# tjhladish/PLS

Hardware: AMD Instinct MI355X
Metric: NIPALS components/sec (higher is better)
Workload: dtype f64; 1 GPU; C3: synthetic tall n=1048576 x p=512, m=1, A=20, f64, resident in HBM; algo=nipals, fuse=1, deflation_written_back_every=1, rows_per_gpu=1048576, parallelism=single GPU

## Files before the change

pls_amd/csrc/ctx.hpp:

```cpp
#pragma once

namespace {

struct DevBuf {
    void *p = nullptr;
    size_t bytes = 0;
};

struct Launch {
    int fam;
    i64 bytes;
    hipEvent_t e0, e1;
};

}

struct pls_hip_context {
    int device = 0;
    hipStream_t stream = nullptr;
    pls_hip_allreduce_fn reducer = nullptr;
    void *reducer_user = nullptr;
    int rank = 0, nranks = 1;
    double *user_red = nullptr;
    i64 user_red_count = 0;
// ... 17 lines not shown
    i64 opt_val_lds_rows = -1;
    i64 val_lds_rows_dev = -1;
    std::string err;
    std::vector<hipEvent_t> ev_pool;
    size_t ev_used = 0;
    std::vector<Launch> launches;
    std::vector<Launch> fits;
    Launch cur_fit{};
    bool fit_timed = false;
    int num_cu = 256;
    plsh::Stager stager;
    int copy_threads = 0;
    hipStream_t copy_stream = nullptr;
    const double *pre_xx = nullptr, *pre_xy = nullptr;
    bool defer_free = false;
    std::vector<void *> graveyard;
    struct XchgIpc *xchg = nullptr;
    struct XchgEndpoint {
        bool on = false;
        int n = 0, rank = 0;
        double *const *inbox = nullptr;
        unsigned long long *const *flags = nullptr;
        unsigned long long *seq = nullptr;
        int *status = nullptr, *host_status = nullptr;
        const long long *limit = nullptr;
    } xep;
    DevBuf tailcnt;
    DevBuf resident;
    DevBuf rgflags;
    unsigned rg_epoch = 0;
    unsigned long long resident_launches = 0;
    struct Env {
        bool turnaround = true;
        i64 turn_edge_bytes = plsk::TURN_EDGE_BYTES;
        bool batch_refit = false;
        i64 batch_round = 0;
        i64 dualcv_round = 0;
        i64 dualbatch_round = 0;
        i64 resample_round = 0;
        bool resample_refit = false;
        bool dualbatch_sweeps = false;
        bool cvbatch_refit = false;
        i64 dualcvb_round = 0;
        i64 misscv_round = 0;
        bool tiny = true, cv_refit = false, tail = true, replica_guard = true, resident = true;
        int tail_update = 1;
        int xb4 = 1;
        int resident_gram = 1;
    };
    static void read_env(Env &env) {
        auto off = [](const char *name) { const char *e = getenv(name); return e && atoi(e) == 0; };
        auto on = [](const char *name) { const char *e = getenv(name); return e && atoi(e) != 0; };
        auto num = [](const char *name, i64 &v) { if (const char *e = getenv(name)) v = atoll(e); };
        env.tiny = !off("PLS_HIP_TINY");
        env.cv_refit = on("PLS_HIP_CV_REFIT");
        env.batch_refit = on("PLS_HIP_BATCH_REFIT");
        num("PLS_HIP_BATCH_ROUND", env.batch_round);
        num("PLS_HIP_DUALCV_ROUND", env.dualcv_round);
        num("PLS_HIP_DUALBATCH_ROUND", env.dualbatch_round);
        num("PLS_HIP_RESAMPLE_ROUND", env.resample_round);
        env.resample_refit = on("PLS_HIP_RESAMPLE_REFIT");
        env.dualbatch_sweeps = on("PLS_HIP_DUALBATCH_SWEEPS");
        env.cvbatch_refit = on("PLS_HIP_CVBATCH_REFIT");
        num("PLS_HIP_DUALCVB_ROUND", env.dualcvb_round);
        num("PLS_HIP_MISSCV_ROUND", env.misscv_round);
        env.tail = !off("PLS_HIP_TAIL");
        const char *tail = getenv("PLS_HIP_TAIL");
        env.tail_update = tail ? (atoi(tail) >= 2 ? 2 : 0) : 1;
        env.replica_guard = !off("PLS_HIP_REPLICA_GUARD");
        env.resident = !off("PLS_HIP_RESIDENT");
        env.turnaround = !off("PLS_HIP_TURNAROUND");
#ifdef PLS_HIP_TESTING
        num("PLS_HIP_TEST_TURN_EDGE_BYTES", env.turn_edge_bytes);
#endif
        if (const char *e = getenv("PLS_HIP_XB4")) env.xb4 = atoi(e);
        if (const char *e = getenv("PLS_HIP_RESIDENT_GRAM")) env.resident_gram = atoi(e);
    }
    Env env;
    int *diverged = nullptr, *diverged_dev = nullptr;
    DevBuf guard;
#ifdef PLS_HIP_TESTING
    int poison_new = -1;
#endif
};

#define PLS_HIP_WORKSPACES(SCRATCH, STATEFUL)                                                                                        \
    STATEFUL(zeros, WS_ALL, "256 zero bytes, cleared once when first used and only read afterwards: the source of out-of-range rows of the LDS-DMA panels") \
    STATEFUL(resident, 256, "two arrival counters of the resident fits, used in alternating parity (resident_launches): each launch zeroes the counter of the next; the payload behind the 256 bytes is scratch") \
    STATEFUL(rgflags, WS_ALL, "one arrival word per workgroup of resident_gram_fit_kernel: values only grow, a launch waits for words beyond rg_epoch, which the host advances by 4 per launch") \
    STATEFUL(gxx, c->pre_xx ? WS_ALL : 0, "X^T X accumulated during an upload, only while pre_xx points into it: from upload_accumulate to the end of the same host-memory fit") \
    STATEFUL(gxy, c->pre_xy ? WS_ALL : 0, "X^T Y accumulated during an upload, only while pre_xy points into it: from upload_accumulate to the end of the same host-memory fit") \
    SCRATCH(tailcnt) SCRATCH(part) SCRATCH(sspart) SCRATCH(xbpart) SCRATCH(wide1) SCRATCH(red) SCRATCH(red2) SCRATCH(xx) SCRATCH(xyp)  \
    SCRATCH(praw) SCRATCH(xy) SCRATCH(v) SCRATCH(cs) SCRATCH(coop) SCRATCH(lm) SCRATCH(tab) SCRATCH(work)                              \
    SCRATCH(cvidx) SCRATCH(cvx) SCRATCH(cvy) SCRATCH(cvws) SCRATCH(cve) SCRATCH(cvtx) SCRATCH(cvty) SCRATCH(cvtt) SCRATCH(cvm)         \
    SCRATCH(cvkeep) SCRATCH(cvred)                                                                                                     \
    SCRATCH(hX) SCRATCH(hY) SCRATCH(hT) SCRATCH(hW) SCRATCH(hP) SCRATCH(hQ) SCRATCH(hR) SCRATCH(hB) SCRATCH(hIn) SCRATCH(hOut)         \
    SCRATCH(valout) SCRATCH(valpart) SCRATCH(vale) SCRATCH(valacc) SCRATCH(valkeys) SCRATCH(valhist)                                   \
    SCRATCH(xdS) SCRATCH(xdQ) SCRATCH(xdPT) SCRATCH(xdred) SCRATCH(xdtv) SCRATCH(xdoQ) SCRATCH(xdoT) SCRATCH(xdoS) SCRATCH(xdsmall)    \
    SCRATCH(bws) SCRATCH(bv) SCRATCH(bred) SCRATCH(bmsg) SCRATCH(bssy) SCRATCH(bY) SCRATCH(boR) SCRATCH(boQ) SCRATCH(bott)             \
    SCRATCH(boB) SCRATCH(bossy)                                                                                                        \
    SCRATCH(dG) SCRATCH(dpart) SCRATCH(dV) SCRATCH(dT) SCRATCH(dY) SCRATCH(dZ) SCRATCH(dC) SCRATCH(dscr) SCRATCH(dcv) SCRATCH(dbat)    \
    SCRATCH(dcvb) SCRATCH(cvbpos) SCRATCH(cvbidx) SCRATCH(cvbo) SCRATCH(cvboE)                                                         \
    SCRATCH(rsw) SCRATCH(rsB) SCRATCH(rsacc) SCRATCH(rsX) SCRATCH(rsY) SCRATCH(rsW) SCRATCH(rsoS)                                      \
    SCRATCH(mX) SCRATCH(mws) SCRATCH(mit) SCRATCH(mzo) SCRATCH(mcv) SCRATCH(mcvidx)                                                    \
    SCRATCH(guard)

namespace {

constexpr size_t WS_ALL = ~(size_t)0;

template <typename F>
void for_each_workspace(pls_hip_context *c, F &&f) {
#define PLS_HIP_WS_SCRATCH(name) f(c->name, (size_t)0);
#define PLS_HIP_WS_STATEFUL(name, keep, reason) f(c->name, (size_t)(keep));
    PLS_HIP_WORKSPACES(PLS_HIP_WS_SCRATCH, PLS_HIP_WS_STATEFUL)
// ... 129 lines not shown
```

pls_amd/csrc/fused_kernels.hpp:

```cpp
#pragma once
#include <type_traits>

#include "common.hpp"
#include "exchange_kernels.hpp"
#include "update_m1.hpp"

namespace plsk {

#ifdef PLS_HIP_TESTING
__device__ unsigned long long *g_pass_stamps = nullptr;
#define PLS_STAMP(slot)                                                                                 \
    do {                                                                                                \
        if (g_pass_stamps && threadIdx.x == 0) {                                                        \
            g_pass_stamps[(size_t)blockIdx.x * 8 + (slot)] = wall_clock64();                            \
            if ((slot) == 0) {         \
                g_pass_stamps[(size_t)blockIdx.x * 8 + 4] = __builtin_amdgcn_s_getreg((31 << 11) | 20);  \
                g_pass_stamps[(size_t)blockIdx.x * 8 + 5] = __builtin_amdgcn_s_getreg((31 << 11) | 4);   \
            }                                                                                           \
        }                                                                                               \
    } while (0)
#else
#define PLS_STAMP(slot) do { } while (0)
#endif

// ... 34 lines not shown
template <typename T, int V>
__device__ __forceinline__ Pack<T, V> ld_pack_u(const T *p) {
    Pack<T, V> o;
    __builtin_memcpy(&o, p, sizeof(o));
    return o;
}
template <typename T, int V>
__device__ __forceinline__ void st_pack_u(T *p, const Pack<T, V> &x) {
    __builtin_memcpy(p, &x, sizeof(x));
}

template <typename T>
__device__ __forceinline__ __amdgpu_buffer_rsrc_t score_rsrc(const T *col, i64 nvalid) {
    return __builtin_amdgcn_make_buffer_rsrc(const_cast<T *>(col), (short)0, (int)(nvalid * (i64)sizeof(T)), BUF_WORD3);
}

struct TailUpdate {
    double *XY = nullptr;
    double *W = nullptr, *P = nullptr, *Q = nullptr, *R = nullptr, *vnext = nullptr;
    int A = 0, a = 0, nipals = 0;
};

struct WalkWeights {
    int nfull = -1;
    unsigned mask = 0;
    int rev = 0;
    int edge = 0;
};

struct Turn {
    bool on = false;
    bool rev = false;
    i64 edge_bytes = 0;
};

#ifdef PLS_HIP_TESTING
struct TurnRecord {
    int rev = 0, edge = 0, ntiles = 0, grid = 0;
};
inline TurnRecord g_test_turn;
#endif

struct SliceTail {
    unsigned *cnt = nullptr;
    double *red = nullptr;
    int nrows = 0;
    int npush = 0;
    unsigned long long seq = 0;
    XchgPeers peers;
    TailUpdate upd;
    XchgGather gx;
};

constexpr int TAIL_MIN_WG = 32;
constexpr int TAIL_AUX_SYS = 17;

__device__ __noinline__ void tail_update_m1(const double *src, i64 stride, int n, int sys, int ok, double *XY, double *W, double *P,
                                            double *Q, double *R, double *vnext, int K, int A, int a, int nipals, double *scratch,
                                            double *wl) {
    typedef unsigned int u32x2 __attribute__((ext_vector_type(2)));
    static_assert(XCHG_MAX == 2 * RED_SLICES, "two batches of RED_SLICES loads");
    const int L = K + 1;
    update_m1<512, 1>(
        [&](int j) -> double {
            double sum = 0.0;
#pragma unroll
// ... 129 lines not shown
    }
    if (!st.upd.XY) return;
    const TailUpdate &u = st.upd;
    if (st.gx.n > 0) {
        const XchgGather &gx = st.gx;
        if (tid == 0) *role = (*gx.status == 0);
        __syncthreads();
        if (tid < gx.n && *role) {
            const long long t0 = wall_clock64();
            while (__hip_atomic_load(gx.flags + tid, __ATOMIC_RELAXED, __HIP_MEMORY_SCOPE_SYSTEM) < gx.seq) {
                if (wall_clock64() - t0 > gx.limit) {
                    *role = 0;
                    break;
                }
                __builtin_amdgcn_s_sleep(4);
            }
            __builtin_amdgcn_fence(__ATOMIC_ACQUIRE, "");
            asm volatile("s_waitcnt vmcnt(0)" ::: "memory");
        }
        __syncthreads();
        const int ok = *role;
        if (!ok && tid == 0) {
            *gx.status = 1;
            __hip_atomic_store(gx.host_status, 1, __ATOMIC_RELAXED, __HIP_MEMORY_SCOPE_SYSTEM);
        }
        tail_update_m1(gx.inbox, gx.cap, gx.n, 1, ok, u.XY, u.W, u.P, u.Q, u.R, u.vnext, K, u.A, u.a, u.nipals, scratch, wl);
        return;
    }
    tail_update_m1(st.red, LP, RED_SLICES, 0, 1, u.XY, u.W, u.P, u.Q, u.R, u.vnext, K, u.A, u.a, u.nipals, scratch, wl);
}

constexpr int AUX_NT = 2;
constexpr i64 TURN_EDGE_BYTES = 192ll << 20;
constexpr bool TURN_LEAD_ST_DEFAULT = true;

template <bool XCD, int R>
struct TileWalk {
    __device__ __forceinline__ explicit TileWalk(i64) {}
    __device__ __forceinline__ unsigned first() const { return blockIdx.x; }
    __device__ __forceinline__ unsigned step() const { return gridDim.x; }
    __device__ __forceinline__ i64 nlim(i64 N) const { return N; }
};
template <int R>
struct TileWalk<true, R> {
    i64 first_, step_, nlim_;
    __device__ __forceinline__ explicit TileWalk(i64 N) : first_(blockIdx.x), step_(gridDim.x), nlim_(N) {
        if ((gridDim.x & 7) == 0) {
            const i64 per = ((N + R - 1) / R + 7) / 8;
            first_ = (i64)(blockIdx.x & 7) * per + (blockIdx.x >> 3);
            step_ = gridDim.x >> 3;
            nlim_ = min(N, (i64)((blockIdx.x & 7) + 1) * per * R);
        }
    }
    __device__ __forceinline__ i64 first() const { return first_; }
    __device__ __forceinline__ i64 step() const { return step_; }
    __device__ __forceinline__ i64 nlim(i64) const { return nlim_; }
};

template <typename T, int V, int R, int NT, int CPT, bool DEFL, int LDAUX_ = AUX_NT, int STAUX = AUX_NT, bool RDST = false,
          int EDGE = 0, bool TILED = false, bool ONEWG = false, bool STORE = true>
__global__ __launch_bounds__(NT, (NT / 256) * ((CPT <= 16 && !DEFL && !ONEWG) ? 2 : 1)) void fused_pass_kernel(
    const T *X, i64 ldx, i64 tsx, T *dst, i64 ldd, i64 tsd, i64 N, int K,
    const double *__restrict__ v, const T *__restrict__ tprev, const double *__restrict__ pprev,
    T *__restrict__ tout, double *__restrict__ part, double *__restrict__ sspart, int rdst, i64 NV, const SliceTail st,
    const WalkWeights wk) {
    constexpr int RP = R / V;
    constexpr int CG = NT / RP;
    constexpr int NW = NT / WAVE;
    constexpr int LDAUX = (EDGE == 2) ? 0 : LDAUX_;
    static_assert(RP <= WAVE && WAVE % RP == 0 && NT % RP == 0, "tile shape");
    static_assert(!TILED || (EDGE == 0 && !RDST), "the tiled copy is aligned and keeps one tile shape");
    static_assert(STORE || (DEFL && !RDST), "only a deflating pass has a store side to drop; without it there is no destination tile shape");
    constexpr bool DYN = (size_t)2 * CG * CPT * sizeof(double) > 48 * 1024;
    struct alignas(16) Lds {
        alignas(16) double ps[(DEFL && !DYN) ? CG * CPT : 2];
        alignas(16) double vs[DYN ? 2 : CG * CPT];
        alignas(16) double tred[2][NW][R];
        alignas(16) double sred[NW];
    };
    __shared__ Lds lds;
    extern __shared__ double fused_dyn[];
    double *vs = DYN ? fused_dyn : lds.vs, *ps = DYN ? fused_dyn + CG * CPT : lds.ps;
    auto &tred = lds.tred;
    double *sred = lds.sred;

    const int tid = threadIdx.x, lane = tid & 63, wv = tid >> 6;
    const int rp = tid % RP, cg = tid / RP;
    PLS_STAMP(0);
    constexpr bool LATE_OK = TILED && DEFL && CG * CPT <= NT;
    const bool LATE_FILL = LATE_OK && (rdst & 0x10000);
    double v_late = 0.0, p_late = 0.0;
    if (LATE_FILL) {
        if (tid < CG * CPT) {
            v_late = (tid < K) ? v[tid] : 0.0;
            p_late = (tid < K) ? pprev[tid] : 0.0;
        }
    } else {
        for (int k = tid; k < CG * CPT; k += NT) {
            vs[k] = (k < K) ? v[k] : 0.0;
            if (DEFL) ps[k] = (k < K) ? pprev[k] : 0.0;
        }
        __syncthreads();
    }
    bool first_tile = true;

    double pacc[CPT];
#pragma unroll
    for (int j = 0; j < CPT; ++j) pacc[j] = 0.0;
    double ss = 0.0;
    int buf = 0;
    constexpr int CGD = EDGE ? WAVE / RP : CG;
    const int cgw = EDGE ? __builtin_amdgcn_readfirstlane(cg) : 0;
    const uint32_t xoff = (uint32_t)(((i64)rp * V + (i64)(cg - cgw) * ldx) * (i64)sizeof(T));
    uint32_t doff = (DEFL && STORE) ? (uint32_t)(((i64)rp * V + (i64)cg * ldd) * (i64)sizeof(T)) : 0u;
    i64 dtile = tsd;
    if constexpr (RDST && DEFL) {
        doff = (uint32_t)(((i64)((rp * V) / rdst) * tsd + (rp * V) % rdst + (i64)cg * ldd) * (i64)sizeof(T));
        dtile = (R / rdst) * tsd;
    }
    constexpr uint32_t OOR = 0x80000000u;
    constexpr bool TBUF = DEFL && sizeof(T) == 8 && R == 32 && CPT == 16;
    const __amdgpu_buffer_rsrc_t rs_tin = score_rsrc<T>(DEFL ? tprev : tout, NV);

    TileWalk<EDGE == 2, R> walk(N);
    const int pace = rdst & 0xffff;
    constexpr bool WEIGHTED = DEFL && EDGE != 2;
    const int wfast = (WEIGHTED && wk.nfull >= 0) ? ((wk.mask >> (blockIdx.x & 7)) & 1) : 0;
    const i64 wswitch = (WEIGHTED && wk.nfull >= 0) ? (i64)wk.nfull * gridDim.x : (i64)1 << 62;
    i64 wstep = walk.step();
    bool wshared = true;
    constexpr bool TURNS = DEFL;
    constexpr bool EDGES = TILED && DEFL && STORE;
    const bool rev = TURNS && wk.rev;
    const i64 ntl = (N + R - 1) / R;
    const i64 etrail = ntl - wk.edge;
    for (i64 pos = walk.first(); pos * R < walk.nlim(N); buf ^= 1) {
        const i64 tile = rev ? ntl - 1 - pos : pos;
        if constexpr (EDGES) {
            if (pos < wk.edge) {
                constexpr int LA = 0, SA = TURN_LEAD_ST_DEFAULT ? 0 : STAUX;
#include "fused_pass_tile.inc"
            } else if (pos >= etrail) {
                constexpr int LA = 0, SA = 0;
#include "fused_pass_tile.inc"
            } else {
                constexpr int LA = LDAUX, SA = STAUX;
#include "fused_pass_tile.inc"
            }
        } else {
            constexpr int LA = LDAUX, SA = STAUX;
#include "fused_pass_tile.inc"
        }
        if constexpr (!WEIGHTED) {
            pos += walk.step();
            continue;
        }
        pos += wstep;
        if (wshared && pos >= wswitch) {
            if (!wfast) break;
            wshared = false;
            const int nfc = __builtin_popcount(wk.mask), below = __builtin_popcount(wk.mask & ((1u << (blockIdx.x & 7)) - 1u));
            pos = wswitch + (i64)(blockIdx.x >> 3) * nfc + below;
            wstep = (i64)(gridDim.x >> 3) * nfc;
        }
    }

    PLS_STAMP(1);
#pragma unroll
    for (int j = 0; j < CPT; ++j) {
        const double s = xor_range_sum<1, RP>(pacc[j]);
        const int k = cg + CG * j;
        if (rp == 0 && k < K) st_agent(part + (i64)blockIdx.x * K + k, s);
    }
    ss = block_sum<NW>(ss, sred);
    if (tid == 0) st_agent(sspart + blockIdx.x, ss);
    constexpr bool ONE_PER_CU = !(CPT <= 16 && !DEFL) || ONEWG;
    if (ONE_PER_CU && st.cnt) {
        asm volatile("s_waitcnt vmcnt(0)" ::: "memory");
        __syncthreads();
        static_assert(NT == 512, "tail_update_m1 plays the update's 1024 virtual threads with 512");
        PLS_STAMP(2);
        slice_tail<NT>(st, part, sspart, K, reinterpret_cast<int *>(sred + NW - 1), sred, &tred[0][0][0], vs);
    }
    PLS_STAMP(3);
}

template <typename T, int V, int R, int NT, int CPT, int EDGE = 0>
__global__ __launch_bounds__(NT, (NT / 256) * 2) void deflate_score_kernel(
    const T *src, i64 lds_, i64 tss, T *dst, i64 ldd, i64 tsd, int rdst, i64 N, int K, const T *__restrict__ tprev,
    const double *__restrict__ pprev, const double *__restrict__ w, T *__restrict__ tout,
    double *__restrict__ sspart, i64 NV) {
    constexpr int RP = R / V, CG = NT / RP, NW = NT / WAVE;
    extern __shared__ double dyn[];
    __shared__ double tred[2][NW][R];
    __shared__ double sred[NW];
    double *ws = dyn, *ps = dyn + K;
    const int tid = threadIdx.x, lane = tid & 63, wv = tid >> 6;
    const int rp = tid % RP, cg = tid / RP;
    for (int k = tid; k < K; k += NT) {
        ws[k] = w[k];
        ps[k] = pprev[k];
    }
    __syncthreads();
    constexpr int CGD = EDGE ? WAVE / RP : CG;
    constexpr int LDAUX = (EDGE == 2) ? 0 : AUX_NT;
    const int cgw = EDGE ? __builtin_amdgcn_readfirstlane(cg) : 0;
    const uint32_t soff = (uint32_t)(((i64)rp * V + (i64)(cg - cgw) * lds_) * (i64)sizeof(T));
    const int dsub = (rp * V) / rdst, dwithin = (rp * V) % rdst, dtiles = R / rdst;
    const uint32_t doff = (uint32_t)(((i64)dsub * tsd + dwithin + (i64)cg * ldd) * (i64)sizeof(T));
    constexpr uint32_t OOR = 0x80000000u;
    const int ngroups = (K + CG - 1) / CG;
    const __amdgpu_buffer_rsrc_t rs_tin = score_rsrc<T>(tprev, NV);
    double ss = 0.0;
    int buf = 0;
    TileWalk<EDGE == 2, R> walk(N);
    for (i64 tile = walk.first(); tile * R < walk.nlim(N); tile += walk.step(), buf ^= 1) {
        const i64 i0 = tile * R + (i64)rp * V;
// ... 550 lines not shown
            st = *tail;
            st.nrows = (int)grid + (Nf < N ? 1 : 0);
            if (tail_used) *tail_used = true;
            if (st.upd.XY && upd_done && K <= UPD1_VTHREADS && 2 * (NT / WAVE) * R >= UPD1_VWAVES + st.upd.A) {
                *upd_done = true;
            } else {
                st.upd.XY = nullptr;
                st.gx.n = 0;
            }
        }
        if (Nf < N) {
            TailArgs<T> a;
            a.src = X; a.lds = ldx; a.tss = tsx; a.rs = R;
            if (defl) {
                if (stores) { a.dst = dst; a.ldd = ldd; a.tsd = tsd; a.rd = rdst > 0 ? rdst : R; }
                a.tprev = tprev; a.pprev = pprev;
            }
            a.v = v; a.tout = tout; a.part = part + grid * K; a.sspart = sspart + grid;
            a.row0 = Nf; a.nrows = (int)(N - Nf); a.K = K; a.zero_rows = V - a.nrows;
            launch_tail_rows(stream, a);
        }
        const bool tiled = defl && edge == 0 && rdst == 0 && ldx == R && tsx == (i64)R * K && (!stores || (ldd == R && tsd == (i64)R * K));
        WalkWeights wk;
        {
            constexpr double rho = 1.08;
            constexpr unsigned fast_mask = 0x55u;
            const int nfc = __builtin_popcount(fast_mask);
            if (defl && per_cu == 1 && grid == (i64)num_cu && grid % 8 == 0 && edge != 2 && ntiles >= 2 * grid) {
                const double share = (double)ntiles / ((double)grid * (1.0 + (rho - 1.0) * nfc / 8.0));
                wk.nfull = (int)std::max<i64>(1, std::min<i64>((i64)(share + 0.5), ntiles / grid));
                wk.mask = fast_mask;
            }
        }
        if (turn.on && defl) {
            wk.rev = turn.rev ? 1 : 0;
            if (tiled) {
                const i64 round_bytes = grid * (i64)R * K * (i64)sizeof(T);
                const i64 epos = turn.edge_bytes / round_bytes * grid;
                wk.edge = (int)(2 * epos >= ntiles ? ntiles : epos);
            }
        }
#ifdef PLS_HIP_TESTING
        if (stores) g_test_turn = TurnRecord{wk.rev, wk.edge, (int)ntiles, (int)grid};
#endif
        if (CGX > 32 && defl && !tiled) return 1;
#define FUSED_LAUNCH(CPT_, DEFL_, EDGE_, TILED_, STORE_, dyn_)                                                            \
    do {                                                                                                                  \
        if constexpr (!(DEFL_) && (CPT_) <= 16 && CGX <= 64 && (EDGE_) == 0) {                                            \
            if (onewg) {                                                                                                  \
                auto kfn1 = &fused_pass_kernel<T, V, R, NT, CPT_, DEFL_, AUX_NT, AUX_NT, false, EDGE_, TILED_, true>;     \
                hipLaunchKernelGGL(kfn1, g, b, dyn_, stream, X, ldx, tsx, dst, ldd, tsd, Nf, K, v, tprev, pprev, tout, part, sspart, 0, N, st, wk); \
                break;                                                                                                    \
            }                                                                                                             \
        }                                                                                                                 \
        auto kfn = &fused_pass_kernel<T, V, R, NT, CPT_, DEFL_, AUX_NT, AUX_NT, false, EDGE_, TILED_, false, STORE_>;    \
        if ((dyn_) > 48 * 1024 && !raise_dynamic_lds(reinterpret_cast<const void *>(kfn), (int)(dyn_))) return 1;         \
        hipLaunchKernelGGL(kfn, g, b, dyn_, stream, X, ldx, tsx, dst, ldd, tsd, Nf, K, v, tprev, pprev, tout, part, sspart, (TILED_) ? ((STORE_) ? 2 * (CPT_) : 0) | 0x10000 : 0, N, st, wk); \
    } while (0)
#define FUSED_EDGE(CPT_, DEFL_, STORE_, dyn_)                                                                             \
    do {                                                                                                                  \
        if constexpr (DEFL_) {                                                                                            \
            if (tiled) { FUSED_LAUNCH(CPT_, DEFL_, 0, true, STORE_, dyn_); break; }                                       \
        }                                                                                                                 \
        if constexpr (CGX <= 32) {                                                                                        \
            if (edge == 2) { FUSED_LAUNCH(CPT_, DEFL_, 2, false, STORE_, dyn_); break; }                                  \
            if (edge == 1) { FUSED_LAUNCH(CPT_, DEFL_, 1, false, STORE_, dyn_); break; }                                  \
        }                                                                                                                 \
        if constexpr (CGX <= 32 || !DEFL_) FUSED_LAUNCH(CPT_, DEFL_, 0, false, STORE_, dyn_);                             \
    } while (0)
#define FUSED_CASE(CPT_)                                                                                                  \
    do {                                                                                                                  \
        const size_t dyn = ((size_t)2 * CG * CPT_ * sizeof(double) > 48 * 1024) ? (size_t)2 * CG * CPT_ * sizeof(double) : 0; \
        if (stores) FUSED_EDGE(CPT_, true, true, dyn);                                                                    \
        else if (defl) FUSED_EDGE(CPT_, true, false, dyn);                        \
        else FUSED_EDGE(CPT_, false, true, (CGX >= 512 ? dyn / 2 : dyn));    \
    } while (0)
        if constexpr (CGX == 32) {
            if (rdst > 0) {
                auto kfn = edge == 2 ? &fused_pass_kernel<T, V, R, NT, 32, true, AUX_NT, AUX_NT, true, 2>
                                     : (edge == 1 ? &fused_pass_kernel<T, V, R, NT, 32, true, AUX_NT, AUX_NT, true, 1>
                                                  : &fused_pass_kernel<T, V, R, NT, 32, true, AUX_NT, AUX_NT, true, 0>);
                hipLaunchKernelGGL(kfn, g, b, 0, stream, X, ldx, tsx, dst, ldd, tsd, Nf, K, v, tprev, pprev, tout, part, sspart, rdst, N, st, wk);
            } else if (K <= CG * 4) FUSED_CASE(4);
            else if (K <= CG * 8) FUSED_CASE(8);
            else if (K <= CG * 12) FUSED_CASE(12);
            else if (K <= CG * 16) FUSED_CASE(16);
            else if (K <= CG * 24) FUSED_CASE(24);
            else FUSED_CASE(32);
        } else if constexpr (CGX == 64 || CGX == 128) {
            if (K <= CG * 12) FUSED_CASE(12);
            else FUSED_CASE(16);
        } else if constexpr (CGX == 8) {
            if (K <= CG * 4) FUSED_CASE(4);
            else if (K <= CG * 8) FUSED_CASE(8);
            else if (K <= CG * 12) FUSED_CASE(12);
// ... 37 lines not shown
```

pls_amd/csrc/fused_pass_tile.inc:

```
        const i64 i0 = tile * R + (i64)rp * V;
        const bool rowok = (i0 < N);
        const uint32_t xo = rowok ? xoff : OOR, dof = rowok ? doff : OOR;
        int cgz = cg;
        asm volatile("" : "+v"(cgz));
        if constexpr (TILED && DEFL && STORE) {
            if (!LATE_FILL || !first_tile)
                for (int q = 0; q < pace; ++q) __builtin_amdgcn_s_sleep(1);
        }
        Pack<T, V> x[CPT];
        constexpr int GSTEP = CG * R * (int)sizeof(T);
        const int trec = K * R * (int)sizeof(T);
        if constexpr (TILED) {
            const __amdgpu_buffer_rsrc_t rs =
                __builtin_amdgcn_make_buffer_rsrc(const_cast<T *>(X + tile * tsx), (short)0, trec, BUF_WORD3);
#pragma unroll
            for (int j = 0; j < CPT; ++j) x[j] = buf_ld_so<T, V, LA>(rs, xo, j * GSTEP);
            __builtin_amdgcn_sched_barrier(0);
            if constexpr (LATE_OK) {
                if (LATE_FILL && first_tile) {
                    first_tile = false;
                    if (tid < CG * CPT) {
                        vs[tid] = v_late;
                        ps[tid] = p_late;
                    }
                    __syncthreads();
                }
            }
        } else {
#pragma unroll
            for (int j = 0; j < CPT; ++j) {
                const int cols = min(CGD, K - CG * j - cgw);
                const uint32_t nrec = cols > 0 ? (uint32_t)((i64)cols * ldx * (i64)sizeof(T)) : 0u;
                const __amdgpu_buffer_rsrc_t rs = __builtin_amdgcn_make_buffer_rsrc(
                    const_cast<T *>(X + tile * tsx + (i64)(j * CG + cgw) * ldx), (short)0, (int)nrec, BUF_WORD3);
                x[j] = buf_ld<T, V, LA>(rs, xo);
                __builtin_amdgcn_sched_barrier(0);
            }
        }
        if (DEFL) {
            double tp[V];
            {
                Pack<T, V> tpk;
                if constexpr (TBUF) {
                    tpk = buf_ld<T, V>(rs_tin, rowok ? (uint32_t)(i0 * (i64)sizeof(T)) : OOR);
                } else if (rowok && i0 + V <= NV) {
                    tpk = ld_pack_u<T, V>(tprev + i0);
                } else {
#pragma unroll
                    for (int e = 0; e < V; ++e) tpk.v[e] = (rowok && i0 + e < NV) ? tprev[i0 + e] : (T)0;
                }
#pragma unroll
                for (int e = 0; e < V; ++e) tp[e] = -(double)tpk.v[e];
            }
#pragma unroll
            for (int j = 0; j < CPT; ++j) {
                const double pk = ps[cgz + CG * j];
#pragma unroll
                for (int e = 0; e < V; ++e) x[j].v[e] = (T)fma(tp[e], pk, (double)x[j].v[e]);
                if constexpr (!STORE) {
                    continue;
                } else if constexpr (TILED) {
                    const __amdgpu_buffer_rsrc_t rd =
                        __builtin_amdgcn_make_buffer_rsrc(dst + tile * tsd, (short)0, trec, BUF_WORD3);
                    buf_st_so<T, V, SA>(rd, dof, j * GSTEP, x[j]);
                } else if constexpr (RDST) {
                    const __amdgpu_buffer_rsrc_t rd = __builtin_amdgcn_make_buffer_rsrc(
                        dst + tile * dtile + (i64)j * CG * ldd, (short)0, 0x7fffffff, BUF_WORD3);
                    buf_st<T, V, SA>(rd, (cg + CG * j < K) ? dof : OOR, x[j]);
                } else {
                    const int cols = min(CG, K - CG * j);
                    const uint32_t nrec = cols > 0 ? (uint32_t)((i64)cols * ldd * (i64)sizeof(T)) : 0u;
                    const __amdgpu_buffer_rsrc_t rd = __builtin_amdgcn_make_buffer_rsrc(
                        dst + tile * tsd + (i64)j * CG * ldd, (short)0, (int)nrec, BUF_WORD3);
                    buf_st<T, V, SA>(rd, dof, x[j]);
                }
            }
        }
        if constexpr (DEFL && STORE) __builtin_amdgcn_sched_barrier(0);
        double tp2[V];
#pragma unroll
        for (int e = 0; e < V; ++e) tp2[e] = 0.0;
#pragma unroll
        for (int j = 0; j < CPT; ++j) {
            const double vk = vs[cgz + CG * j];
#pragma unroll
            for (int e = 0; e < V; ++e) tp2[e] = fma((double)x[j].v[e], vk, tp2[e]);
        }
#pragma unroll
        for (int e = 0; e < V; ++e)
            tp2[e] = xor_range_sum<RP, WAVE>(tp2[e]);
        if (lane < RP)
#pragma unroll
            for (int e = 0; e < V; ++e) tred[buf][wv][rp * V + e] = tp2[e];
        __syncthreads();
// ... 33 lines not shown
```

pls_amd/csrc/plan_fit.hpp:

```cpp
#pragma once

namespace {

template <typename T>
struct FitWork {
    double *red, *part, *sspart, *XY, *v;
    T *work;
    plsk::SliceTail tail;
    bool retiled = false;
    bool xx_local_done = false;
    int nip;
};

template <typename T>
int fit_workspace(pls_hip_context *c, const plsk::FitShape &shape, plsk::FitPlan &plan, FitWork<T> &w) {
    CHK(ensure(c, c->part, plan.part_bytes));
    CHK(ensure(c, c->sspart, plan.sspart_bytes));
    CHK(ensure(c, c->xy, (size_t)shape.K * shape.M * 8));
    CHK(ensure(c, c->v, (size_t)shape.K * 8));
    CHK(ensure(c, c->cs, (size_t)shape.A * 8));
    if (c->user_red) {
        if (c->user_red_count < (i64)(plan.red_bytes / 8)) return fail(c, PLS_HIP_ERR_INVALID, "reduce buffer too small");
        w.red = c->user_red;
    } else {
        CHK(ensure(c, c->red, plan.red_bytes));
        w.red = (double *)c->red.p;
    }
    if (plan.retile_fit && ensure(c, c->work, plan.work_bytes) != PLS_HIP_OK) {
        c->err.clear();
        plan = plsk::fit_plan(shape, plsk::FIT_NO_COPY);
    }
    if (plan.work_bytes) CHK(ensure(c, c->work, plan.work_bytes));
    w.part = (double *)c->part.p;
    w.sspart = (double *)c->sspart.p;
    w.XY = (double *)c->xy.p;
    w.v = (double *)c->v.p;
    w.work = (T *)c->work.p;
    if (c->env.tail && c->opt_fuse && shape.N > 0) {
        if (!c->tailcnt.p) CHK(ensure(c, c->tailcnt, 256));
        HIPCHK(c, hipMemsetAsync(c->tailcnt.p, 0, 256, c->stream));
        w.tail.cnt = (unsigned *)c->tailcnt.p;
        w.tail.red = w.red;
    }
    w.nip = plan.algo == plsk::FIT_NIPALS ? 1 : 0;
    return PLS_HIP_OK;
}

template <typename T>
int fit_xty(pls_hip_context *c, const FitArgs<T> &f, const plsk::FitPlan &p, FitWork<T> &w) {
    const T *X = f.X;
    const i64 N = f.N, ldx = f.ldx;
    const int K = f.K, M = f.M;
    const i64 L0 = (i64)K * M;
    const bool type2 = p.algo == plsk::FIT_GRAM || p.algo == plsk::FIT_TYPE2;
    Range r_phase("X^T Y");
    if (!p.use_pre && N > 0 && (p.retile_fit || p.nip_copy) && M <= 8) {
        int nb = 0, rc = 1;
        {
            Scope s(c, PLS_HIP_FAM_DEFLATE, 2 * (i64)N * K * sizeof(T) + (i64)N * M * sizeof(T) + L0 * 8);
            rc = pick_int<8, 16, 32>(p.fused_mode ? p.tall_cg : 32, [&](auto cg) {
                return plsk::launch_retile_xty<T, decltype(cg)::value>(c->stream, c->num_cu, X, ldx, f.Y, f.ldy, w.work, p.WR, p.WR * (i64)K, (int)p.WR, N, K,
                                                                       M, w.part, (int)p.prow, &nb);
            });
            if (rc != 0) s.on = false;
        }
        if (rc == 0) {
            LAUNCH_CHECK(c);
            CHK(launch_reduce(c, w.part, nb, (int)L0, nullptr, 0, w.red));
            w.retiled = true;
        }
// ... 239 lines not shown
        CHK(launch_xty<T>(c, st.Xc, st.ldc, f.Tm + (i64)a * f.ldt, f.ldt, N, K, 1, w.part, &nb));
    }
    CHK(launch_reduce(c, w.part, nb, K, w.sspart, nss, w.red));
    return PLS_HIP_OK;
}

inline plsk::XchgGather exchange_gather(const pls_hip_context *c, unsigned long long seq) {
    const int par = (int)(seq & 1);
    plsk::XchgGather gx;
    gx.inbox = c->xep.inbox[c->xep.rank] + (i64)par * c->xep.n * plsk::XCHG_CAP;
    gx.flags = c->xep.flags[c->xep.rank] + par * c->xep.n;
    gx.n = c->xep.n; gx.cap = plsk::XCHG_CAP; gx.seq = seq;
    gx.status = c->xep.status; gx.host_status = c->xep.host_status; gx.limit = *c->xep.limit;
    return gx;
}

template <typename T>
int fit_passes(pls_hip_context *c, const FitArgs<T> &f, const plsk::FitPlan &p, FitWork<T> &w) {
    const i64 N = f.N;
    const int K = f.K, M = f.M, A = f.A;
    plsk::SliceTail &tail = w.tail;
    PassState<T> st;
    st.Xc = f.X;
    st.ldc = f.ldx;
    st.tsc = p.TR;
    using Route = int (*)(pls_hip_context *, const FitArgs<T> &, const plsk::FitPlan &, FitWork<T> &, PassState<T> &, int);
    const Route routes[] = {pass_deferred<T>, pass_tall<T>, pass_short_tile<T>, pass_unfused<T>};
    for (int a = 0; a < A; ++a) {
        Range r_comp("component", a);
        st.tail_used = st.upd_done = false;
        const bool want_push = tail.cnt && p.xep_ok && update_is_single(K, M, A, a);
        const bool defl_pass = w.nip && a > 0;
        st.store_x = (a + 1 < A);
        st.turn = plsk::Turn{c->env.turnaround, c->env.turnaround && a % 2 == 0, c->env.turn_edge_bytes};
        const bool want_upd = tail.cnt && (c->env.tail_update == 2 || (c->env.tail_update == 1 && !defl_pass)) && M == 1 &&
                              K <= plsk::UPD1_KMAX && update_is_single(K, M, A, a) && (!c->reducer || want_push);
        tail.npush = 0;
        tail.upd = plsk::TailUpdate();
        tail.gx = plsk::XchgGather();
        if (want_push) {
            const unsigned long long seq = *c->xep.seq + 1;
            const int par = (int)(seq & 1);
            tail.npush = c->xep.n;
            tail.seq = seq;
            for (int j = 0; j < c->xep.n; ++j) {
                tail.peers.slot[j] = c->xep.inbox[j] + ((i64)par * c->xep.n + c->xep.rank) * plsk::XCHG_CAP;
                tail.peers.flag[j] = c->xep.flags[j] + par * c->xep.n + c->xep.rank;
            }
            if (want_upd) tail.gx = exchange_gather(c, seq);
        }
        if (want_upd) {
            tail.upd.XY = w.XY; tail.upd.W = f.W; tail.upd.P = f.P; tail.upd.Q = f.Q; tail.upd.R = f.R; tail.upd.vnext = w.v;
            tail.upd.A = A; tail.upd.a = a; tail.upd.nipals = w.nip;
        }
        if (N > 0) {
            int rc = PASS_NOT_COVERED;
            for (Route route : routes)
                if ((rc = route(c, f, p, w, st, a)) != PASS_NOT_COVERED) break;
            CHK(rc);
        } else {
            HIPCHK(c, hipMemsetAsync(w.red, 0, (size_t)plsk::RED_SLICES * (K + 1) * 8, c->stream));
        }
        if (st.upd_done) {
            if (want_push) ++*c->xep.seq;
        } else if (st.tail_used && want_push) {
            const plsk::XchgGather gx = exchange_gather(c, ++*c->xep.seq);
            CHK(launch_update(c, w.red, w.XY, f.W, f.P, f.Q, f.R, w.v, K, M, A, a, w.nip, &gx));
// ... 38 lines not shown
```

pls_amd/csrc/pls_hip.hip:

```cpp
#include <dlfcn.h>
#include <unistd.h>
#include <hip/hip_runtime.h>

#include <algorithm>
#include <atomic>
#include <cstdio>
#include <cstring>
#include <memory>
#include <new>
#include <string>
#include <type_traits>
#include <vector>

#include "../../include/pls_hip.h"
#include "fused_kernels.hpp"
#include "defer_kernels.hpp"
#include "small_kernels.hpp"
#include "coop_update.hpp"
#include "wide1_update.hpp"
#include "largem_kernels.hpp"
#include "tiny_kernels.hpp"
#include "resident_kernels.hpp"
#include "resident_gram.hpp"
#include "stream_kernels.hpp"
// ... 37 lines not shown
#include "plan_batch.hpp"
#include "plan_resample.hpp"
#include "plan_dual_cvbatch.hpp"
#include "plan_missing.hpp"
#include "plan_missing_cv.hpp"
#include "xchg_ipc.hpp"
#include "group_impl.hpp"

extern "C" {

int pls_hip_abi_version(void) { return PLS_HIP_ABI_VERSION; }

#ifdef PLS_HIP_TESTING
__attribute__((visibility("default"))) int pls_hip_test_set_pass_stamps(void *buf) {
    unsigned long long *p = (unsigned long long *)buf;
    return hipMemcpyToSymbol(HIP_SYMBOL(plsk::g_pass_stamps), &p, sizeof(p)) == hipSuccess ? 0 : 1;
}
__attribute__((visibility("default"))) int pls_hip_test_last_turn(int *out) {
    if (!out) return 1;
    out[0] = plsk::g_test_turn.rev; out[1] = plsk::g_test_turn.edge; out[2] = plsk::g_test_turn.ntiles; out[3] = plsk::g_test_turn.grid;
    return 0;
}
__attribute__((visibility("default"))) long long pls_hip_test_poison_workspace(pls_hip_handle h, int byte, int also_new) {
    if (!h || hipSetDevice(h->device) != hipSuccess || hipStreamSynchronize(h->stream) != hipSuccess) return -1;
    long long filled = 0;
    bool ok = true;
    for_each_workspace(h, [&](DevBuf &b, size_t keep) {
        if (!b.p || keep >= b.bytes) return;
        ok = ok && hipMemsetAsync((char *)b.p + keep, byte & 0xFF, b.bytes - keep, h->stream) == hipSuccess;
        filled += (long long)(b.bytes - keep);
    });
    h->poison_new = also_new ? (byte & 0xFF) : -1;
    return ok && hipStreamSynchronize(h->stream) == hipSuccess ? filled : -1;
}
#endif

int pls_hip_create(pls_hip_handle *out, int device, void *stream) {
    if (!out) return PLS_HIP_ERR_INVALID;
    *out = nullptr;
    int ndev = 0;
    if (hipGetDeviceCount(&ndev) != hipSuccess || ndev <= 0 || device < 0 || device >= ndev) {
        (void)hipGetLastError();
        return PLS_HIP_ERR_DEVICE;
    }
    hipDeviceProp_t prop;
    if (hipGetDeviceProperties(&prop, device) != hipSuccess) return PLS_HIP_ERR_DEVICE;
    if (std::strncmp(prop.gcnArchName, "gfx950", 6) != 0) return PLS_HIP_ERR_DEVICE;
    pls_hip_context *c = new (std::nothrow) pls_hip_context();
    if (!c) return PLS_HIP_ERR_ALLOC;
    pls_hip_context::read_env(c->env);
    c->device = device;
    c->num_cu = prop.multiProcessorCount > 0 ? prop.multiProcessorCount : 256;
    if (hipSetDevice(device) != hipSuccess) { delete c; return PLS_HIP_ERR_DEVICE; }
    c->stream = (hipStream_t)stream;
    *out = c;
    return PLS_HIP_OK;
}

int pls_hip_destroy(pls_hip_handle h) {
    if (!h) return PLS_HIP_OK;
    (void)hipSetDevice(h->device);
    (void)hipStreamSynchronize(h->stream);
    for_each_workspace(h, [](DevBuf &b, size_t) {
        if (b.p) (void)hipFree(b.p);
    });
    for (void *q : h->graveyard) (void)hipFree(q);
// ... 708 lines not shown
```

Before: 755.9 components/s.

## Write first deflation directly into tiled workspace layout with turnaround edges

Adds a dedicated first-deflation kernel that reads X from aligned columns and stores the deflated copy straight into the R-row tiled workspace layout. Subsequent passes can then use the faster tiled path instead of a column layout. It also applies the turnaround edge logic, with non-temporal store flags dropped on trailing edge tiles so those tiles stay cache-resident for the next reversed pass. The kernel body is moved into a shared include file, and test-only guard bands are added around the workspace to detect out-of-range writes.

```diff
diff --git a/pls_amd/csrc/ctx.hpp b/pls_amd/csrc/ctx.hpp
--- a/pls_amd/csrc/ctx.hpp
+++ b/pls_amd/csrc/ctx.hpp
@@ -73,6 +73,7 @@
     unsigned long long resident_launches = 0;
     struct Env {
         bool turnaround = true;
+        bool first_defl_tiled = true;
         i64 turn_edge_bytes = plsk::TURN_EDGE_BYTES;
         bool batch_refit = false;
         i64 batch_round = 0;
@@ -111,6 +112,7 @@
         env.replica_guard = !off("PLS_HIP_REPLICA_GUARD");
         env.resident = !off("PLS_HIP_RESIDENT");
         env.turnaround = !off("PLS_HIP_TURNAROUND");
+        env.first_defl_tiled = !off("PLS_HIP_FIRST_DEFL_TILED");
 #ifdef PLS_HIP_TESTING
         num("PLS_HIP_TEST_TURN_EDGE_BYTES", env.turn_edge_bytes);
 #endif
@@ -122,6 +124,8 @@
     DevBuf guard;
 #ifdef PLS_HIP_TESTING
     int poison_new = -1;
+    size_t work_guard = 0, work_inner = 0;
+    static constexpr int WORK_GUARD_BYTE = 0xA5;
 #endif
 };
 
diff --git a/pls_amd/csrc/fused_kernels.hpp b/pls_amd/csrc/fused_kernels.hpp
--- a/pls_amd/csrc/fused_kernels.hpp
+++ b/pls_amd/csrc/fused_kernels.hpp
@@ -90,6 +90,7 @@
     bool on = false;
     bool rev = false;
     i64 edge_bytes = 0;
+    bool first_tiled = true;
 };
 
 #ifdef PLS_HIP_TESTING
@@ -285,6 +286,10 @@
 
 constexpr int AUX_NT = 2;
 constexpr i64 TURN_EDGE_BYTES = 192ll << 20;
+#ifndef PLS_HIP_FIRST_DEFL_PACE
+#define PLS_HIP_FIRST_DEFL_PACE 0
+#endif
+constexpr int FIRST_DEFL_PACE = PLS_HIP_FIRST_DEFL_PACE;
 constexpr bool TURN_LEAD_ST_DEFAULT = true;
 
 template <bool XCD, int R>
@@ -317,125 +322,18 @@
     const double *__restrict__ v, const T *__restrict__ tprev, const double *__restrict__ pprev,
     T *__restrict__ tout, double *__restrict__ part, double *__restrict__ sspart, int rdst, i64 NV, const SliceTail st,
     const WalkWeights wk) {
-    constexpr int RP = R / V;
-    constexpr int CG = NT / RP;
-    constexpr int NW = NT / WAVE;
-    constexpr int LDAUX = (EDGE == 2) ? 0 : LDAUX_;
-    static_assert(RP <= WAVE && WAVE % RP == 0 && NT % RP == 0, "tile shape");
-    static_assert(!TILED || (EDGE == 0 && !RDST), "the tiled copy is aligned and keeps one tile shape");
-    static_assert(STORE || (DEFL && !RDST), "only a deflating pass has a store side to drop; without it there is no destination tile shape");
-    constexpr bool DYN = (size_t)2 * CG * CPT * sizeof(double) > 48 * 1024;
-    struct alignas(16) Lds {
-        alignas(16) double ps[(DEFL && !DYN) ? CG * CPT : 2];
-        alignas(16) double vs[DYN ? 2 : CG * CPT];
-        alignas(16) double tred[2][NW][R];
-        alignas(16) double sred[NW];
-    };
-    __shared__ Lds lds;
-    extern __shared__ double fused_dyn[];
-    double *vs = DYN ? fused_dyn : lds.vs, *ps = DYN ? fused_dyn + CG * CPT : lds.ps;
-    auto &tred = lds.tred;
-    double *sred = lds.sred;
-
-    const int tid = threadIdx.x, lane = tid & 63, wv = tid >> 6;
-    const int rp = tid % RP, cg = tid / RP;
-    PLS_STAMP(0);
-    constexpr bool LATE_OK = TILED && DEFL && CG * CPT <= NT;
-    const bool LATE_FILL = LATE_OK && (rdst & 0x10000);
-    double v_late = 0.0, p_late = 0.0;
-    if (LATE_FILL) {
-        if (tid < CG * CPT) {
-            v_late = (tid < K) ? v[tid] : 0.0;
-            p_late = (tid < K) ? pprev[tid] : 0.0;
-        }
-    } else {
-        for (int k = tid; k < CG * CPT; k += NT) {
-            vs[k] = (k < K) ? v[k] : 0.0;
-            if (DEFL) ps[k] = (k < K) ? pprev[k] : 0.0;
-        }
-        __syncthreads();
-    }
-    bool first_tile = true;
-
-    double pacc[CPT];
-#pragma unroll
-    for (int j = 0; j < CPT; ++j) pacc[j] = 0.0;
-    double ss = 0.0;
-    int buf = 0;
-    constexpr int CGD = EDGE ? WAVE / RP : CG;
-    const int cgw = EDGE ? __builtin_amdgcn_readfirstlane(cg) : 0;
-    const uint32_t xoff = (uint32_t)(((i64)rp * V + (i64)(cg - cgw) * ldx) * (i64)sizeof(T));
-    uint32_t doff = (DEFL && STORE) ? (uint32_t)(((i64)rp * V + (i64)cg * ldd) * (i64)sizeof(T)) : 0u;
-    i64 dtile = tsd;
-    if constexpr (RDST && DEFL) {
-        doff = (uint32_t)(((i64)((rp * V) / rdst) * tsd + (rp * V) % rdst + (i64)cg * ldd) * (i64)sizeof(T));
-        dtile = (R / rdst) * tsd;
-    }
-    constexpr uint32_t OOR = 0x80000000u;
-    constexpr bool TBUF = DEFL && sizeof(T) == 8 && R == 32 && CPT == 16;
-    const __amdgpu_buffer_rsrc_t rs_tin = score_rsrc<T>(DEFL ? tprev : tout, NV);
-
-    TileWalk<EDGE == 2, R> walk(N);
-    const int pace = rdst & 0xffff;
-    constexpr bool WEIGHTED = DEFL && EDGE != 2;
-    const int wfast = (WEIGHTED && wk.nfull >= 0) ? ((wk.mask >> (blockIdx.x & 7)) & 1) : 0;
-    const i64 wswitch = (WEIGHTED && wk.nfull >= 0) ? (i64)wk.nfull * gridDim.x : (i64)1 << 62;
-    i64 wstep = walk.step();
-    bool wshared = true;
-    constexpr bool TURNS = DEFL;
-    constexpr bool EDGES = TILED && DEFL && STORE;
-    const bool rev = TURNS && wk.rev;
-    const i64 ntl = (N + R - 1) / R;
-    const i64 etrail = ntl - wk.edge;
-    for (i64 pos = walk.first(); pos * R < walk.nlim(N); buf ^= 1) {
-        const i64 tile = rev ? ntl - 1 - pos : pos;
-        if constexpr (EDGES) {
-            if (pos < wk.edge) {
-                constexpr int LA = 0, SA = TURN_LEAD_ST_DEFAULT ? 0 : STAUX;
-#include "fused_pass_tile.inc"
-            } else if (pos >= etrail) {
-                constexpr int LA = 0, SA = 0;
-#include "fused_pass_tile.inc"
-            } else {
-                constexpr int LA = LDAUX, SA = STAUX;
-#include "fused_pass_tile.inc"
-            }
-        } else {
-            constexpr int LA = LDAUX, SA = STAUX;
-#include "fused_pass_tile.inc"
-        }
-        if constexpr (!WEIGHTED) {
-            pos += walk.step();
-            continue;
-        }
-        pos += wstep;
-        if (wshared && pos >= wswitch) {
-            if (!wfast) break;
-            wshared = false;
-            const int nfc = __builtin_popcount(wk.mask), below = __builtin_popcount(wk.mask & ((1u << (blockIdx.x & 7)) - 1u));
-            pos = wswitch + (i64)(blockIdx.x >> 3) * nfc + below;
-            wstep = (i64)(gridDim.x >> 3) * nfc;
-        }
-    }
-
-    PLS_STAMP(1);
-#pragma unroll
-    for (int j = 0; j < CPT; ++j) {
-        const double s = xor_range_sum<1, RP>(pacc[j]);
-        const int k = cg + CG * j;
-        if (rp == 0 && k < K) st_agent(part + (i64)blockIdx.x * K + k, s);
-    }
-    ss = block_sum<NW>(ss, sred);
-    if (tid == 0) st_agent(sspart + blockIdx.x, ss);
-    constexpr bool ONE_PER_CU = !(CPT <= 16 && !DEFL) || ONEWG;
-    if (ONE_PER_CU && st.cnt) {
-        asm volatile("s_waitcnt vmcnt(0)" ::: "memory");
-        __syncthreads();
-        static_assert(NT == 512, "tail_update_m1 plays the update's 1024 virtual threads with 512");
-        PLS_STAMP(2);
-        slice_tail<NT>(st, part, sspart, K, reinterpret_cast<int *>(sred + NW - 1), sred, &tred[0][0][0], vs);
-    }
-    PLS_STAMP(3);
+    constexpr bool DTILED = false;
+#include "fused_pass_body.inc"
+}
+
+template <typename T, int V, int R, int NT, int CPT>
+__global__ __launch_bounds__(NT, NT / 256) void fused_first_deflation_kernel(
+    const T *X, i64 ldx, i64 tsx, T *dst, i64 ldd, i64 tsd, i64 N, int K, const double *__restrict__ v,
+    const T *__restrict__ tprev, const double *__restrict__ pprev, T *__restrict__ tout, double *__restrict__ part,
+    double *__restrict__ sspart, int rdst, i64 NV, const SliceTail st, const WalkWeights wk) {
+    constexpr bool DEFL = true, RDST = false, TILED = false, ONEWG = false, STORE = true, DTILED = true;
+    constexpr int LDAUX_ = AUX_NT, STAUX = AUX_NT, EDGE = 0;
+#include "fused_pass_body.inc"
 }
 
 template <typename T, int V, int R, int NT, int CPT, int EDGE = 0>
@@ -1052,9 +950,10 @@
                 wk.mask = fast_mask;
             }
         }
+        const bool dtiled = stores && turn.first_tiled && CGX <= 32 && !tiled && edge == 0 && rdst == 0 && ldd == R && tsd == (i64)R * K;
         if (turn.on && defl) {
             wk.rev = turn.rev ? 1 : 0;
-            if (tiled) {
+            if (tiled || dtiled) {
                 const i64 round_bytes = grid * (i64)R * K * (i64)sizeof(T);
                 const i64 epos = turn.edge_bytes / round_bytes * grid;
                 wk.edge = (int)(2 * epos >= ntiles ? ntiles : epos);
@@ -1081,6 +980,13 @@
     do {                                                                                                                  \
         if constexpr (DEFL_) {                                                                                            \
             if (tiled) { FUSED_LAUNCH(CPT_, DEFL_, 0, true, STORE_, dyn_); break; }                                       \
+        }                                                                                                                 \
+        if constexpr ((DEFL_) && (STORE_) && CGX <= 32) {                                                                 \
+            if (dtiled) {                                                                                                 \
+                auto kfn0 = &fused_first_deflation_kernel<T, V, R, NT, CPT_>;                                             \
+                hipLaunchKernelGGL(kfn0, g, b, dyn_, stream, X, ldx, tsx, dst, ldd, tsd, Nf, K, v, tprev, pprev, tout, part, sspart, FIRST_DEFL_PACE * (CPT_), N, st, wk); \
+                break;                                                                                                    \
+            }                                                                                                             \
         }                                                                                                                 \
         if constexpr (CGX <= 32) {                                                                                        \
             if (edge == 2) { FUSED_LAUNCH(CPT_, DEFL_, 2, false, STORE_, dyn_); break; }                                  \
diff --git a/pls_amd/csrc/fused_pass_body.inc b/pls_amd/csrc/fused_pass_body.inc
--- /dev/null
+++ b/pls_amd/csrc/fused_pass_body.inc
@@ -0,0 +1,128 @@
+    constexpr int RP = R / V;
+    constexpr int CG = NT / RP;
+    constexpr int NW = NT / WAVE;
+    constexpr int LDAUX = (EDGE == 2) ? 0 : LDAUX_;
+    static_assert(RP <= WAVE && WAVE % RP == 0 && NT % RP == 0, "tile shape");
+    static_assert(!TILED || (EDGE == 0 && !RDST), "the tiled copy is aligned and keeps one tile shape");
+    static_assert(STORE || (DEFL && !RDST), "only a deflating pass has a store side to drop; without it there is no destination tile shape");
+    static_assert(!DTILED || (DEFL && STORE && EDGE == 0 && !RDST && !TILED), "the first deflation from aligned columns into this tile shape");
+    constexpr bool DYN = (size_t)2 * CG * CPT * sizeof(double) > 48 * 1024;
+    struct alignas(16) Lds {
+        alignas(16) double ps[(DEFL && !DYN) ? CG * CPT : 2];
+        alignas(16) double vs[DYN ? 2 : CG * CPT];
+        alignas(16) double tred[2][NW][R];
+        alignas(16) double sred[NW];
+    };
+    __shared__ Lds lds;
+    extern __shared__ double fused_dyn[];
+    double *vs = DYN ? fused_dyn : lds.vs, *ps = DYN ? fused_dyn + CG * CPT : lds.ps;
+    auto &tred = lds.tred;
+    double *sred = lds.sred;
+
+    const int tid = threadIdx.x, lane = tid & 63, wv = tid >> 6;
+    const int rp = tid % RP, cg = tid / RP;
+    PLS_STAMP(0);
+    constexpr bool LATE_OK = TILED && DEFL && CG * CPT <= NT;
+    const bool LATE_FILL = LATE_OK && (rdst & 0x10000);
+    double v_late = 0.0, p_late = 0.0;
+    if (LATE_FILL) {
+        if (tid < CG * CPT) {
+            v_late = (tid < K) ? v[tid] : 0.0;
+            p_late = (tid < K) ? pprev[tid] : 0.0;
+        }
+    } else {
+        for (int k = tid; k < CG * CPT; k += NT) {
+            vs[k] = (k < K) ? v[k] : 0.0;
+            if (DEFL) ps[k] = (k < K) ? pprev[k] : 0.0;
+        }
+        __syncthreads();
+    }
+    bool first_tile = true;
+
+    double pacc[CPT];
+#pragma unroll
+    for (int j = 0; j < CPT; ++j) pacc[j] = 0.0;
+    double ss = 0.0;
+    int buf = 0;
+    constexpr int CGD = EDGE ? WAVE / RP : CG;
+    const int cgw = EDGE ? __builtin_amdgcn_readfirstlane(cg) : 0;
+    const uint32_t xoff = (uint32_t)(((i64)rp * V + (i64)(cg - cgw) * ldx) * (i64)sizeof(T));
+    uint32_t doff = (DEFL && STORE) ? (uint32_t)(((i64)rp * V + (i64)cg * ldd) * (i64)sizeof(T)) : 0u;
+    i64 dtile = tsd;
+    if constexpr (RDST && DEFL) {
+        doff = (uint32_t)(((i64)((rp * V) / rdst) * tsd + (rp * V) % rdst + (i64)cg * ldd) * (i64)sizeof(T));
+        dtile = (R / rdst) * tsd;
+    }
+    constexpr uint32_t OOR = 0x80000000u;
+    constexpr bool TBUF = DEFL && sizeof(T) == 8 && R == 32 && CPT == 16;
+    const __amdgpu_buffer_rsrc_t rs_tin = score_rsrc<T>(DEFL ? tprev : tout, NV);
+
+    TileWalk<EDGE == 2, R> walk(N);
+    const int pace = rdst & 0xffff;
+    constexpr bool WEIGHTED = DEFL && EDGE != 2;
+    const int wfast = (WEIGHTED && wk.nfull >= 0) ? ((wk.mask >> (blockIdx.x & 7)) & 1) : 0;
+    const i64 wswitch = (WEIGHTED && wk.nfull >= 0) ? (i64)wk.nfull * gridDim.x : (i64)1 << 62;
+    i64 wstep = walk.step();
+    bool wshared = true;
+    constexpr bool TURNS = DEFL;
+    constexpr bool EDGES = TILED && DEFL && STORE;
+    const bool rev = TURNS && wk.rev;
+    const i64 ntl = (N + R - 1) / R;
+    const i64 etrail = ntl - wk.edge;
+    for (i64 pos = walk.first(); pos * R < walk.nlim(N); buf ^= 1) {
+        const i64 tile = rev ? ntl - 1 - pos : pos;
+        if constexpr (EDGES) {
+            if (pos < wk.edge) {
+                constexpr int LA = 0, SA = TURN_LEAD_ST_DEFAULT ? 0 : STAUX;
+#include "fused_pass_tile.inc"
+            } else if (pos >= etrail) {
+                constexpr int LA = 0, SA = 0;
+#include "fused_pass_tile.inc"
+            } else {
+                constexpr int LA = LDAUX, SA = STAUX;
+#include "fused_pass_tile.inc"
+            }
+        } else if constexpr (DTILED) {
+            if (pos >= etrail) {
+                constexpr int LA = LDAUX, SA = 0;
+#include "fused_pass_tile.inc"
+            } else {
+                constexpr int LA = LDAUX, SA = STAUX;
+#include "fused_pass_tile.inc"
+            }
+        } else {
+            constexpr int LA = LDAUX, SA = STAUX;
+#include "fused_pass_tile.inc"
+        }
+        if constexpr (!WEIGHTED) {
+            pos += walk.step();
+            continue;
+        }
+        pos += wstep;
+        if (wshared && pos >= wswitch) {
+            if (!wfast) break;
+            wshared = false;
+            const int nfc = __builtin_popcount(wk.mask), below = __builtin_popcount(wk.mask & ((1u << (blockIdx.x & 7)) - 1u));
+            pos = wswitch + (i64)(blockIdx.x >> 3) * nfc + below;
+            wstep = (i64)(gridDim.x >> 3) * nfc;
+        }
+    }
+
+    PLS_STAMP(1);
+#pragma unroll
+    for (int j = 0; j < CPT; ++j) {
+        const double s = xor_range_sum<1, RP>(pacc[j]);
+        const int k = cg + CG * j;
+        if (rp == 0 && k < K) st_agent(part + (i64)blockIdx.x * K + k, s);
+    }
+    ss = block_sum<NW>(ss, sred);
+    if (tid == 0) st_agent(sspart + blockIdx.x, ss);
+    constexpr bool ONE_PER_CU = !(CPT <= 16 && !DEFL) || ONEWG;
+    if (ONE_PER_CU && st.cnt) {
+        asm volatile("s_waitcnt vmcnt(0)" ::: "memory");
+        __syncthreads();
+        static_assert(NT == 512, "tail_update_m1 plays the update's 1024 virtual threads with 512");
+        PLS_STAMP(2);
+        slice_tail<NT>(st, part, sspart, K, reinterpret_cast<int *>(sred + NW - 1), sred, &tred[0][0][0], vs);
+    }
+    PLS_STAMP(3);
diff --git a/pls_amd/csrc/fused_pass_tile.inc b/pls_amd/csrc/fused_pass_tile.inc
--- a/pls_amd/csrc/fused_pass_tile.inc
+++ b/pls_amd/csrc/fused_pass_tile.inc
@@ -3,7 +3,7 @@
         const uint32_t xo = rowok ? xoff : OOR, dof = rowok ? doff : OOR;
         int cgz = cg;
         asm volatile("" : "+v"(cgz));
-        if constexpr (TILED && DEFL && STORE) {
+        if constexpr ((TILED || DTILED) && DEFL && STORE) {
             if (!LATE_FILL || !first_tile)
                 for (int q = 0; q < pace; ++q) __builtin_amdgcn_s_sleep(1);
         }
@@ -59,7 +59,7 @@
                 for (int e = 0; e < V; ++e) x[j].v[e] = (T)fma(tp[e], pk, (double)x[j].v[e]);
                 if constexpr (!STORE) {
                     continue;
-                } else if constexpr (TILED) {
+                } else if constexpr (TILED || DTILED) {
                     const __amdgpu_buffer_rsrc_t rd =
                         __builtin_amdgcn_make_buffer_rsrc(dst + tile * tsd, (short)0, trec, BUF_WORD3);
                     buf_st_so<T, V, SA>(rd, dof, j * GSTEP, x[j]);
diff --git a/pls_amd/csrc/plan_fit.hpp b/pls_amd/csrc/plan_fit.hpp
--- a/pls_amd/csrc/plan_fit.hpp
+++ b/pls_amd/csrc/plan_fit.hpp
@@ -26,16 +26,27 @@
         CHK(ensure(c, c->red, plan.red_bytes));
         w.red = (double *)c->red.p;
     }
-    if (plan.retile_fit && ensure(c, c->work, plan.work_bytes) != PLS_HIP_OK) {
+    size_t lead = 0;
+#ifdef PLS_HIP_TESTING
+    lead = c->work_guard;
+#endif
+    if (plan.retile_fit && ensure(c, c->work, plan.work_bytes + 2 * lead) != PLS_HIP_OK) {
         c->err.clear();
         plan = plsk::fit_plan(shape, plsk::FIT_NO_COPY);
     }
-    if (plan.work_bytes) CHK(ensure(c, c->work, plan.work_bytes));
+    if (plan.work_bytes) CHK(ensure(c, c->work, plan.work_bytes + 2 * lead));
+#ifdef PLS_HIP_TESTING
+    if (lead && plan.work_bytes) {
+        HIPCHK(c, hipMemsetAsync(c->work.p, pls_hip_context::WORK_GUARD_BYTE, lead, c->stream));
+        HIPCHK(c, hipMemsetAsync((char *)c->work.p + lead + plan.work_bytes, pls_hip_context::WORK_GUARD_BYTE, lead, c->stream));
+        c->work_inner = plan.work_bytes;
+    }
+#endif
     w.part = (double *)c->part.p;
     w.sspart = (double *)c->sspart.p;
     w.XY = (double *)c->xy.p;
     w.v = (double *)c->v.p;
-    w.work = (T *)c->work.p;
+    w.work = (T *)((char *)c->work.p + lead);
     if (c->env.tail && c->opt_fuse && shape.N > 0) {
         if (!c->tailcnt.p) CHK(ensure(c, c->tailcnt, 256));
         HIPCHK(c, hipMemsetAsync(c->tailcnt.p, 0, 256, c->stream));
@@ -341,7 +352,7 @@
         const bool want_push = tail.cnt && p.xep_ok && update_is_single(K, M, A, a);
         const bool defl_pass = w.nip && a > 0;
         st.store_x = (a + 1 < A);
-        st.turn = plsk::Turn{c->env.turnaround, c->env.turnaround && a % 2 == 0, c->env.turn_edge_bytes};
+        st.turn = plsk::Turn{c->env.turnaround, c->env.turnaround && a % 2 == 0, c->env.turn_edge_bytes, c->env.first_defl_tiled};
         const bool want_upd = tail.cnt && (c->env.tail_update == 2 || (c->env.tail_update == 1 && !defl_pass)) && M == 1 &&
                               K <= plsk::UPD1_KMAX && update_is_single(K, M, A, a) && (!c->reducer || want_push);
         tail.npush = 0;
diff --git a/pls_amd/csrc/pls_hip.hip b/pls_amd/csrc/pls_hip.hip
--- a/pls_amd/csrc/pls_hip.hip
+++ b/pls_amd/csrc/pls_hip.hip
@@ -93,6 +93,22 @@
     });
     h->poison_new = also_new ? (byte & 0xFF) : -1;
     return ok && hipStreamSynchronize(h->stream) == hipSuccess ? filled : -1;
+}
+__attribute__((visibility("default"))) int pls_hip_test_guard_work(pls_hip_handle h, long long bytes) {
+    if (!h || bytes < 0 || bytes % 256 != 0) return 1;
+    h->work_guard = (size_t)bytes;
+    h->work_inner = 0;
+    return 0;
+}
+__attribute__((visibility("default"))) long long pls_hip_test_work_guard_damage(pls_hip_handle h) {
+    if (!h || !h->work_guard || !h->work_inner || !h->work.p || h->work.bytes < h->work_inner + 2 * h->work_guard) return -1;
+    if (hipSetDevice(h->device) != hipSuccess || hipStreamSynchronize(h->stream) != hipSuccess) return -1;
+    std::vector<unsigned char> g(2 * h->work_guard);
+    if (hipMemcpy(g.data(), h->work.p, h->work_guard, hipMemcpyDeviceToHost) != hipSuccess) return -1;
+    if (hipMemcpy(g.data() + h->work_guard, (char *)h->work.p + h->work_guard + h->work_inner, h->work_guard, hipMemcpyDeviceToHost) != hipSuccess) return -1;
+    long long bad = 0;
+    for (unsigned char b : g) bad += (b != pls_hip_context::WORK_GUARD_BYTE);
+    return bad;
 }
 #endif
 
```

Result: no change. 756.8 components/s, median of 6 (+0.1%).
